# ShengkaiWu/IoU-aware-single-stage-object-detector

Measured on AMD Instinct MI355X. Metric: images/sec at 1333x800, IoU-aware RetinaNet R-50-FPN, higher is better.
Workload: dtype fp32; 1 GPU; IoU-aware RetinaNet R-50-FPN fp32, batch 8 per GPU, 3x800x1344 (1333x800 padded to /32), random-init weights, whole inference path incl. NMS, device-to-host copy and bbox2result (the reference's simple_test: per-class arrays on the host; batch i's host part runs under batch i+1's device part, the last one inside the timed region); global_batch=8, parallelism=dp1, dets_per_image=100

## Files before the change

### include/iouaware.h

```cpp
#ifndef IOUAWARE_H
#define IOUAWARE_H

#include <stddef.h>
#include <stdint.h>

#ifdef __cplusplus
extern "C" {
#endif

#define IA_MAX_LEVELS 8
#define IA_MAX_ANCHORS 16
#define IA_MAX_NMS_PRE 4096
#define IA_MAX_CANDIDATES 8192
#define IA_MAX_PER_IMG 1024

#define IA_F32 0
#define IA_BF16 1
#define IA_F16 2
#define IA_F64 3

#define IA_LAYOUT_NCHW 0
#define IA_LAYOUT_NHWC 1

#define IA_CLS_SIGMOID 0
// ... 53 lines not shown
                     int rescale, float *boxes, float *scores_t, float *best_score, void *stream);

size_t ia_multiclass_nms_workspace_bytes(int batch, int R, int C);
int ia_multiclass_nms(const float *boxes, const float *scores_t, const float *best_score,
                      int batch, int R, int C, float score_thr, float iou_thr, int max_per_img,
                      void *workspace, size_t workspace_bytes, float *dets, int32_t *labels,
                      int32_t *rows, int32_t *num, int32_t *keep_count, int32_t *keep_rows,
                      void *stream);

#define IA_SOFT_LINEAR 1
#define IA_SOFT_GAUSSIAN 2
size_t ia_multiclass_soft_nms_workspace_bytes(int batch, int R, int C);
int ia_multiclass_soft_nms(const float *boxes, const float *scores_t, int batch, int R, int C,
                           float score_thr, float iou_thr, int method, float sigma,
                           float min_score, int max_per_img, void *workspace,
                           size_t workspace_bytes, float *dets, int32_t *labels, int32_t *rows,
                           int32_t *num, int32_t *keep_count, int32_t *keep_rows, void *stream);

size_t ia_get_bboxes_workspace_bytes(const ia_head_geom *g, int batch);
size_t ia_get_bboxes_status_offset(const ia_head_geom *g, int batch);
int ia_debug_fused_spin_limit(int64_t limit);
int ia_profile_stage_events(void *begin, void *end);
int ia_get_bboxes(const ia_head_geom *g, const ia_level_ptrs *p, int batch, int dtype,
                  const float *img_hw, const float *scale_factor, int rescale, float score_thr,
                  float iou_thr, int max_per_img, void *workspace, size_t workspace_bytes,
                  float *dets, int32_t *labels, int32_t *rows, int32_t *num, void *stream);

int ia_get_bboxes_lazy(const ia_head_geom *g, const ia_level_ptrs *p, int batch, int dtype,
                       const float *img_hw, const float *scale_factor, int rescale,
                       float score_thr, float iou_thr, int max_per_img, int candidates,
                       void *workspace, size_t workspace_bytes, float *dets, int32_t *labels,
                       int32_t *rows, int32_t *num, void *stream);

size_t ia_multiclass_nms_lazy_workspace_bytes(int batch, int R, int C);
int ia_multiclass_nms_lazy(const float *boxes, const float *scores_t, const float *best_score,
                           int batch, int R, int C, float score_thr, float iou_thr,
                           int max_per_img, int candidates, void *workspace,
                           size_t workspace_bytes, float *dets, int32_t *labels, int32_t *rows,
                           int32_t *num, void *stream);

int ia_decode_stage(const ia_head_geom *g, const ia_level_ptrs *p, int batch, int dtype,
                    const float *img_hw, const float *scale_factor, int rescale, void *workspace,
                    size_t workspace_bytes, void *stream);

int ia_get_bboxes_workspace_layout(const ia_head_geom *g, int batch, size_t offsets[8]);

size_t ia_nms_workspace_bytes(int n);
int ia_nms(const float *dets, int n, float iou_thr, int32_t *keep, int32_t *count, void *workspace,
           size_t workspace_bytes, void *stream);

size_t ia_nms_f64_workspace_bytes(int n);
int ia_nms_f64(const double *dets, int n, float iou_thr, int32_t *keep, int32_t *count,
               void *workspace, size_t workspace_bytes, void *stream);

int ia_soft_nms(const float *dets, int n, float iou_thr, int method, float sigma, float min_score,
                float *out_dets, int32_t *out_inds, int32_t *count, void *stream);

typedef struct {
    const uint8_t *src;
    int32_t src_h, src_w, dst_h, dst_w, flip;
} ia_image_desc;
int ia_image_transform(const ia_image_desc *imgs, int batch, const float *mean, const float *std,
                       int to_rgb, int pad_h, int pad_w, int channels_last, float *out,
                       void *stream);

typedef struct {
    int32_t num_levels, batch;
    int32_t H[IA_MAX_LEVELS], W[IA_MAX_LEVELS];
} ia_wino_geom;
typedef struct {
    int32_t c0, n;
    int32_t dst_channels, dst_offset;
    float *dst[IA_MAX_LEVELS];
} ia_wino_seg;
int ia_wino_tiles(const ia_wino_geom *g, int32_t *tiles);
int ia_wino_input_transform(const ia_wino_geom *g, const float *const *x, int channels, int groups,
                            const float *pre_scale, const float *pre_shift, int pre_relu, float *V,
                            void *stream);
int ia_wino_output_transform(const ia_wino_geom *g, const float *M, int channels, int groups,
                             const float *bias, int relu, int nseg, const ia_wino_seg *segs,
                             void *stream);
int ia_wino_mid_transform(const ia_wino_geom *g, const float *M, int channels, int groups_m,
                          const float *bias, int relu, float *V, int groups_v, void *stream);

int ia_wino_grad_output_transform(const ia_wino_geom *g, const float *const *dy, int channels,
                                  float *dM, void *stream);

#define IA_COLSUM_MAX_STRIPS 512
size_t ia_relu_bwd_bias_grad_workspace_bytes(int64_t rows, int n);
int ia_wino_weight_transform(const float *w, int n_in, int n_out, int64_t stride_in,
                             int64_t stride_out, int64_t stride_ky, int64_t stride_kx, int flip,
                             const double *G, float *U, void *stream);
int ia_wino_weight_grad(const float *dU, int n_in, int n_out, const double *G, float *dW,
                        int64_t stride_in, int64_t stride_out, int64_t stride_ky, int64_t stride_kx,
                        void *stream);
int ia_bn_fold_fwd(const float *w, const float *gamma, const float *beta, const float *mean,
                   const float *inv_std, int cout, int K, float *w_out, float *b_out, void *stream);
int ia_bn_fold_bwd(const float *dw_folded, const float *db_folded, const float *w, const float *gamma,
                   const float *mean, const float *inv_std, int cout, int K, float *dw,
                   float *dgamma, float *dbeta, void *stream);
int ia_relu_bwd_bias_grad(const float *dy, const float *y, int64_t rows, int n, float *g, float *db,
                          void *workspace, size_t workspace_bytes, void *stream);

int ia_linear_bias_act(const float *A, const float *W, const float *bias, const float *residual,
                       float *D, int64_t rows, int k, int n, int relu, void *workspace,
                       size_t workspace_bytes, void *stream);
int ia_linear_bias_act_bf16(const void *A, const void *W, const float *bias, const void *residual,
                            void *D, int64_t rows, int k, int n, int relu, void *workspace,
                            size_t workspace_bytes, void *stream);
int ia_batched_gemm(const float *A, const float *W, float *D, int batch, int64_t rows, int k, int n,
                    void *workspace, size_t workspace_bytes, void *stream);
int ia_batched_gemm_stream(const float *A, const float *W, float *D, int batch, int64_t rows, int k,
                           int n, void *stream);

size_t ia_im2col3x3_bytes(int B, int H, int W, int C, int stride, int dtype);
int ia_im2col3x3_nhwc(const void *x, void *col, int B, int H, int W, int C, int stride, int dtype,
                      void *stream);
int ia_conv1x1_strided(const void *x, const void *W_kn, const float *bias, const void *residual,
                       void *D, int B, int H, int W, int k, int n, int stride, int relu, int dtype,
                       void *workspace, size_t workspace_bytes, void *stream);
int ia_col2im3x3_nhwc(const void *dcol, void *dx, int B, int H, int W, int C, int stride, int dtype,
                      void *stream);

int ia_gemm_tuning(int mode);

int ia_gemm_table_add(int64_t m, int64_t n, int64_t k, int flags, int batch, int dtype,
                      int solution_index);
int ia_gemm_table_clear(void);
int ia_gemm_table_dump(int64_t *rows7, int capacity);
int ia_gemm_table_stats(int64_t *hits_misses_stale);
int ia_gemm_library_version(void);

int ia_linear_bias_act_wt(const float *A, const float *W_nk, const float *bias,
                          const float *residual, float *D, int64_t rows, int k, int n, int relu,
                          void *workspace, size_t workspace_bytes, void *stream);
int ia_gemm_tn(const float *G, const float *X, float *D, int batch, int64_t rows, int n, int k,
               void *workspace, size_t workspace_bytes, void *stream);


int ia_focal_loss_fwd(const void *cls, int dtype, const int64_t *labels,
                      const float *label_weights, int B, int A, int C, int HW, float gamma,
                      float alpha, double *loss_sum, void *stream);
int ia_focal_loss_bwd(const void *cls, int dtype, const int64_t *labels,
                      const float *label_weights, int B, int A, int C, int HW, float gamma,
                      float alpha, float gscale, const float *gscale_dev, float *grad_cls,
                      void *stream);

int ia_smooth_l1_fwd(const void *pred, int dtype, const float *target, const float *weight,
                     int B, int A, int HW, float beta, double *loss_sum, void *stream);
int ia_smooth_l1_bwd(const void *pred, int dtype, const float *target, const float *weight,
                     int B, int A, int HW, float beta, float gscale, const float *gscale_dev,
                     float *grad_pred, void *stream);

int ia_balanced_l1_fwd(const void *pred, int dtype, const float *target, const float *weight,
                       int B, int A, int HW, float beta, float alpha, float gamma, double *loss_sum,
                       void *stream);
int ia_balanced_l1_bwd(const void *pred, int dtype, const float *target, const float *weight,
                       int B, int A, int HW, float beta, float alpha, float gamma, float gscale,
                       const float *gscale_dev, float *grad_pred, void *stream);

int ia_focal_loss_balanced_fwd(const void *cls, int dtype, const int64_t *labels,
                               const float *label_weights, const float *anchor_iou, int B, int A,
                               int C, int HW, float gamma, float alpha, float eta,
                               double *loss_sums3, void *stream);
int ia_focal_loss_balanced_bwd(const void *cls, int dtype, const int64_t *labels,
                               const float *label_weights, const float *anchor_iou, int B, int A,
// ... 343 lines not shown
```

### iou-aware-single-stage-object-detector_amd/csrc/wino.hip

```cpp
#include <string.h>
#include "ia_internal.hpp"
#include "ia_wino.hpp"

namespace ia {

typedef float f32x4_t __attribute__((ext_vector_type(4)));
__device__ __forceinline__ float4 load_nt(const float *p)
{
    const f32x4_t q = __builtin_nontemporal_load(reinterpret_cast<const f32x4_t *>(p));
    return make_float4(q.x, q.y, q.z, q.w);
}
__device__ __forceinline__ void store_nt(float *p, const float4 &v)
{
    f32x4_t q; q.x = v.x; q.y = v.y; q.z = v.z; q.w = v.w;
    __builtin_nontemporal_store(q, reinterpret_cast<f32x4_t *>(p));
}
__device__ __forceinline__ float4 f4(float v) { return make_float4(v, v, v, v); }
__device__ __forceinline__ float4 operator+(const float4 &a, const float4 &b) { return make_float4(a.x + b.x, a.y + b.y, a.z + b.z, a.w + b.w); }
__device__ __forceinline__ float4 operator-(const float4 &a, const float4 &b) { return make_float4(a.x - b.x, a.y - b.y, a.z - b.z, a.w - b.w); }
__device__ __forceinline__ float4 operator*(float s, const float4 &a) { return make_float4(s * a.x, s * a.y, s * a.z, s * a.w); }

__device__ __forceinline__ void bt6(const float4 (&d)[6], float4 (&o)[6])
{
    o[0] = (4.0f * d[0] - 5.0f * d[2]) + d[4];
// ... 40 lines not shown
    }
    return m;
}
static int tiles_per_wave(int channels)
{
    const int q = channels / 4;
    return (q < 64) ? (64 / q) : 1;
}

template <bool PACKED>
__global__ void __launch_bounds__(64) k_wino_in(WinoInArgs a)
{
    const LaneMap lm = lane_map<PACKED>(a.Ctot, a.T, a.tpw);
    if (!lm.on) return;
    const int t = lm.t, c = lm.c;
    int H, W;
    const TileRef r = locate_tile(a.lv, t, &H, &W);
    const float *x = level_ptr<!PACKED>(a.x, r.l) + (size_t)r.b * H * W * a.Ctot + c;
    const bool pre = a.pre_shift != nullptr;
    float4 ps = f4(1.0f), pb = f4(0.0f);
    if (pre) {
        if (a.pre_scale) ps = *reinterpret_cast<const float4 *>(a.pre_scale + c);
        pb = *reinterpret_cast<const float4 *>(a.pre_shift + c);
    }
    float4 d[6][6];
#pragma unroll
    for (int i = 0; i < 6; ++i) {
        const int y = r.y0 - 1 + i;
        const int yc = (y >= 0 && y < H) ? y : 0;
#pragma unroll
        for (int j = 0; j < 6; ++j) {
            const int xx = r.x0 - 1 + j;
            const int xc = (xx >= 0 && xx < W) ? xx : 0;
            d[i][j] = *reinterpret_cast<const float4 *>(x + ((size_t)yc * W + xc) * a.Ctot);
        }
    }
    if (pre) {
        const bool relu = a.pre_relu != 0;
#pragma unroll
        for (int i = 0; i < 6; ++i)
#pragma unroll
            for (int j = 0; j < 6; ++j) {
                float4 v = d[i][j];
                v = make_float4(v.x * ps.x + pb.x, v.y * ps.y + pb.y, v.z * ps.z + pb.z, v.w * ps.w + pb.w);
                const float4 z = make_float4(v.x > 0.f ? v.x : 0.f, v.y > 0.f ? v.y : 0.f,
                                             v.z > 0.f ? v.z : 0.f, v.w > 0.f ? v.w : 0.f);
                d[i][j] = relu ? z : v;
            }
    }
#pragma unroll
    for (int i = 0; i < 6; ++i) {
        const int y = r.y0 - 1 + i;
        const bool yin = (y >= 0) && (y < H);
#pragma unroll
        for (int j = 0; j < 6; ++j) {
            const int xx = r.x0 - 1 + j;
            const bool in = yin && (xx >= 0) && (xx < W);
            d[i][j] = in ? d[i][j] : f4(0.0f);
        }
    }
    float4 tmp[6][6];
#pragma unroll
    for (int j = 0; j < 6; ++j) {
        float4 col[6], o[6];
#pragma unroll
        for (int i = 0; i < 6; ++i) col[i] = d[i][j];
        bt6(col, o);
#pragma unroll
        for (int i = 0; i < 6; ++i) tmp[i][j] = o[i];
    }
    const int g = c / a.Cg, cc = c - g * a.Cg;
    float *v = a.V + ((size_t)g * 36 * a.T + t) * a.Cg + cc;
    const size_t kstride = (size_t)a.T * a.Cg;
#pragma unroll
    for (int i = 0; i < 6; ++i) {
        float4 o[6];
        bt6(tmp[i], o);
#pragma unroll
        for (int j = 0; j < 6; ++j)
            *reinterpret_cast<float4 *>(v + (size_t)(i * 6 + j) * kstride) = o[j];
    }
}

__device__ __forceinline__ void a6(const float4 (&y)[4], float4 (&o)[6])
{
    const float4 s02 = y[0] + y[2], s13 = y[1] + y[3];
    const float4 t02 = y[0] + 4.0f * y[2], t13 = 2.0f * y[1] + 8.0f * y[3];
    o[0] = y[0];
    o[1] = s02 + s13;
    o[2] = s02 - s13;
    o[3] = t02 + t13;
    o[4] = t02 - t13;
    o[5] = y[3];
}

template <bool PACKED>
__global__ void __launch_bounds__(64) k_wino_dy(WinoInArgs a)
{
    const LaneMap lm = lane_map<PACKED>(a.Ctot, a.T, a.tpw);
    if (!lm.on) return;
    const int t = lm.t, c = lm.c;
    int H, W;
    const TileRef r = locate_tile(a.lv, t, &H, &W);
    const float *x = level_ptr<!PACKED>(a.x, r.l) + (size_t)r.b * H * W * a.Ctot + c;
    float4 d[4][4];
#pragma unroll
    for (int i = 0; i < 4; ++i) {
        const int y = r.y0 + i;
        const int yc = (y < H) ? y : (H - 1);
#pragma unroll
        for (int j = 0; j < 4; ++j) {
            const int xx = r.x0 + j;
            const int xc = (xx < W) ? xx : (W - 1);
            const float4 v = *reinterpret_cast<const float4 *>(x + ((size_t)yc * W + xc) * a.Ctot);
            d[i][j] = (y < H && xx < W) ? v : f4(0.0f);
        }
    }
    float4 tmp[6][4];
#pragma unroll
    for (int j = 0; j < 4; ++j) {
        float4 col[4], o[6];
#pragma unroll
        for (int i = 0; i < 4; ++i) col[i] = d[i][j];
        a6(col, o);
#pragma unroll
        for (int i = 0; i < 6; ++i) tmp[i][j] = o[i];
    }
    const int g = c / a.Cg, cc = c - g * a.Cg;
    float *v = a.V + ((size_t)g * 36 * a.T + t) * a.Cg + cc;
    const size_t kstride = (size_t)a.T * a.Cg;
#pragma unroll
    for (int i = 0; i < 6; ++i) {
        float4 o[6];
        a6(tmp[i], o);
#pragma unroll
        for (int j = 0; j < 6; ++j)
            *reinterpret_cast<float4 *>(v + (size_t)(i * 6 + j) * kstride) = o[j];
    }
}

struct WinoOutArgs {
    WinoLevels lv;
    const float *M;
    const float *bias;
    WinoSeg seg[kMaxSeg];
    int32_t nseg, Ctot, Cg, T, relu, tpw;
};

template <bool PACKED>
__global__ void __launch_bounds__(64) k_wino_out(WinoOutArgs a)
{
    const LaneMap lm = lane_map<PACKED>(a.Ctot, a.T, a.tpw);
    if (!lm.on) return;
    const int t = lm.t, c = lm.c;
    int H, W;
    const TileRef r = locate_tile(a.lv, t, &H, &W);
    const int g = c / a.Cg, cc = c - g * a.Cg;
    const float *m = a.M + ((size_t)g * 36 * a.T + t) * a.Cg + cc;
    const size_t kstride = (size_t)a.T * a.Cg;
    float4 bz = f4(0.0f);
    if (a.bias) bz = *reinterpret_cast<const float4 *>(a.bias + c);
    float4 s[4][6];
#pragma unroll
    for (int j = 0; j < 6; ++j) {
        float4 col[6], o[4];
#pragma unroll
// ... 132 lines not shown
                    const int xx = 4 * txi + j, lx = lx0 + j;
                    float4 v = o[j] + bz;
                    if (a.relu) v = make_float4(v.x > 0.f ? v.x : 0.f, v.y > 0.f ? v.y : 0.f,
                                                v.z > 0.f ? v.z : 0.f, v.w > 0.f ? v.w : 0.f);
                    v = (y < H && xx < W) ? v : f4(0.0f);
                    if (ly >= 0 && ly < kMidP && lx >= 0 && lx < kMidP)
                        *reinterpret_cast<float4 *>(sy + (ly * kMidP + lx) * kMidCh) = v;
                }
            }
        } else {
#pragma unroll
            for (int i = 0; i < 4; ++i)
#pragma unroll
                for (int j = 0; j < 4; ++j) {
                    const int ly = ly0 + i, lx = lx0 + j;
                    if (ly >= 0 && ly < kMidP && lx >= 0 && lx < kMidP)
                        *reinterpret_cast<float4 *>(sy + (ly * kMidP + lx) * kMidCh) = f4(0.0f);
                }
        }
    }
    __syncthreads();

    const int tl = tid / kMidQ, tyl = tl / kMidB, txl = tl - tyl * kMidB;
    const int tyi = kMidB * byi + tyl, txi = kMidB * bxi + txl;
    if (tyi >= ty_n || txi >= tx) return;
    const float *sp = s_y + ((4 * tyl) * kMidP + 4 * txl) * kMidCh + cq;
    float4 tmp[6][6];
#pragma unroll
    for (int j = 0; j < 6; ++j) {
        float4 col[6], o[6];
#pragma unroll
        for (int i = 0; i < 6; ++i) col[i] = *reinterpret_cast<const float4 *>(sp + (i * kMidP + j) * kMidCh);
        bt6(col, o);
#pragma unroll
        for (int i = 0; i < 6; ++i) tmp[i][j] = o[i];
        __builtin_amdgcn_sched_barrier(0);
    }
    float *v = a.V + (size_t)gv * 36 * vstride + (size_t)(tbase + tyi * tx + txi) * a.Cv + (c - gv * a.Cv);
#pragma unroll
    for (int i = 0; i < 6; ++i) {
        float4 o[6];
        bt6(tmp[i], o);
#pragma unroll
        for (int j = 0; j < 6; ++j)
            *reinterpret_cast<float4 *>(v + (size_t)(i * 6 + j) * vstride) = o[j];
    }
}

}

extern "C" {

int ia_wino_tiles(const ia_wino_geom *g, int32_t *tiles)
{
    ia::WinoLevels w;
    int rc = ia::make_wino_levels(g, w);
    if (rc) return rc;
    if (tiles) *tiles = w.tile_off[w.L];
    return 0;
}

int ia_wino_input_transform(const ia_wino_geom *g, const float *const *x, int channels, int groups,
                            const float *pre_scale, const float *pre_shift, int pre_relu, float *V,
                            void *stream)
{
    ia::WinoInArgs a;
    int rc = ia::make_wino_levels(g, a.lv);
    if (rc) return rc;
    if (!x || !V || channels < 4 || (channels & 3) || groups < 1 || channels % groups) return IA_E_ARG;
    a.Ctot = channels; a.Cg = channels / groups; a.T = a.lv.tile_off[a.lv.L];
    if (a.Cg & 3) return IA_E_ARG;
    for (int l = 0; l < IA_MAX_LEVELS; ++l) {
        a.x[l] = (l < a.lv.L) ? x[l] : nullptr;
        if (l < a.lv.L && (!x[l] || ((uintptr_t)x[l] & 15u))) return IA_E_ARG;
    }
    a.V = V;
    if (pre_scale && !pre_shift) return IA_E_ARG;
    a.pre_scale = pre_scale; a.pre_shift = pre_shift; a.pre_relu = pre_relu ? 1 : 0;
    a.tpw = ia::tiles_per_wave(channels);
    const int waves = (a.T + a.tpw - 1) / a.tpw;
    dim3 grid((unsigned)((waves + 7) / 8 * 8), (unsigned)((channels / 4 + 63) / 64));
    if (a.tpw > 1) hipLaunchKernelGGL(ia::k_wino_in<true>, grid, dim3(64), 0, (hipStream_t)stream, a);
    else hipLaunchKernelGGL(ia::k_wino_in<false>, grid, dim3(64), 0, (hipStream_t)stream, a);
    return ia::hip_status(hipGetLastError());
}

int ia_wino_grad_output_transform(const ia_wino_geom *g, const float *const *dy, int channels,
                                   float *dM, void *stream)
{
    ia::WinoInArgs a;
    int rc = ia::make_wino_levels(g, a.lv);
    if (rc) return rc;
    if (!dy || !dM || channels < 4 || (channels & 3)) return IA_E_ARG;
    a.Ctot = channels; a.Cg = channels; a.T = a.lv.tile_off[a.lv.L];
    for (int l = 0; l < IA_MAX_LEVELS; ++l) {
        a.x[l] = (l < a.lv.L) ? dy[l] : nullptr;
        if (l < a.lv.L && (!dy[l] || ((uintptr_t)dy[l] & 15u))) return IA_E_ARG;
    }
    a.V = dM;
    a.pre_scale = a.pre_shift = nullptr; a.pre_relu = 0;
    a.tpw = ia::tiles_per_wave(channels);
    const int waves = (a.T + a.tpw - 1) / a.tpw;
    dim3 grid((unsigned)((waves + 7) / 8 * 8), (unsigned)((channels / 4 + 63) / 64));
    if (a.tpw > 1) hipLaunchKernelGGL(ia::k_wino_dy<true>, grid, dim3(64), 0, (hipStream_t)stream, a);
    else hipLaunchKernelGGL(ia::k_wino_dy<false>, grid, dim3(64), 0, (hipStream_t)stream, a);
    return ia::hip_status(hipGetLastError());
}

int ia_wino_output_transform(const ia_wino_geom *g, const float *M, int channels, int groups,
                             const float *bias, int relu, int nseg, const ia_wino_seg *segs,
                             void *stream)
{
    ia::WinoOutArgs a;
    int rc = ia::make_wino_levels(g, a.lv);
    if (rc) return rc;
    if (!M || channels < 4 || (channels & 3) || groups < 1 || channels % groups || !segs ||
        nseg < 1 || nseg > ia::kMaxSeg)
        return IA_E_ARG;
    a.M = M; a.bias = bias; a.Ctot = channels; a.Cg = channels / groups;
    if (a.Cg & 3) return IA_E_ARG;
    a.T = a.lv.tile_off[a.lv.L]; a.relu = relu ? 1 : 0; a.nseg = nseg;
    memset(a.seg, 0, sizeof(a.seg));
    for (int k = 0; k < nseg; ++k) {
        const ia_wino_seg &s = segs[k];
        if (s.c0 < 0 || s.n < 1 || s.c0 + s.n > channels || s.dst_channels < s.n + s.dst_offset ||
            s.dst_offset < 0)
            return IA_E_ARG;
        if (k > 0 && s.c0 < segs[k - 1].c0 + segs[k - 1].n) return IA_E_ARG;
        a.seg[k].c0 = s.c0; a.seg[k].n = s.n; a.seg[k].Cdst = s.dst_channels; a.seg[k].coff = s.dst_offset;
        for (int l = 0; l < a.lv.L; ++l) {
            if (!s.dst[l]) return IA_E_ARG;
            a.seg[k].dst[l] = s.dst[l];
        }
    }
    a.tpw = ia::tiles_per_wave(channels);
    const int waves = (a.T + a.tpw - 1) / a.tpw;
    dim3 grid((unsigned)((waves + 7) / 8 * 8), (unsigned)((channels / 4 + 63) / 64));
    if (a.tpw > 1) hipLaunchKernelGGL(ia::k_wino_out<true>, grid, dim3(64), 0, (hipStream_t)stream, a);
    else hipLaunchKernelGGL(ia::k_wino_out<false>, grid, dim3(64), 0, (hipStream_t)stream, a);
    return ia::hip_status(hipGetLastError());
}

int ia_wino_mid_transform(const ia_wino_geom *g, const float *M, int channels, int groups_m,
                          const float *bias, int relu, float *V, int groups_v, void *stream)
{
    ia::WinoMidArgs a;
    int rc = ia::make_wino_levels(g, a.lv);
    if (rc) return rc;
    if (!M || !V || channels < ia::kMidCh || groups_m < 1 || channels % groups_m || groups_v < 1 ||
        channels % groups_v)
        return IA_E_ARG;
    a.M = M; a.bias = bias; a.V = V; a.Ctot = channels;
    a.Cm = channels / groups_m; a.Cv = channels / groups_v;
    if (a.Cm % ia::kMidCh || a.Cv % ia::kMidCh || ((uintptr_t)M & 15u) || ((uintptr_t)V & 15u) ||
        ((uintptr_t)bias & 15u))
        return IA_E_ARG;
    a.T = a.lv.tile_off[a.lv.L]; a.relu = relu ? 1 : 0;
    int64_t n = 0;
    for (int l = 0; l < IA_MAX_LEVELS; ++l) {
        const bool on = l < a.lv.L;
        const int ty = on ? a.lv.tpi[l] / a.lv.tx[l] : 0;
        a.bx[l] = on ? (a.lv.tx[l] + ia::kMidB - 1) / ia::kMidB : 0;
        a.bpi[l] = on ? ((ty + ia::kMidB - 1) / ia::kMidB) * a.bx[l] : 0;
        a.blk_off[l] = (int32_t)n;
        n += (int64_t)a.lv.B * a.bpi[l];
    }
// ... 9 lines not shown
```

### iou-aware-single-stage-object-detector_amd/iouaware/_lib.py

```python
import ctypes as C
import os

IA_MAX_LEVELS = 8
IA_MAX_ANCHORS = 16
IA_MAX_NMS_PRE = 4096
IA_MAX_CANDIDATES = 8192
IA_MAX_PER_IMG = 1024
IA_F32, IA_BF16, IA_F16, IA_F64 = 0, 1, 2, 3
IA_LAYOUT_NCHW, IA_LAYOUT_NHWC = 0, 1
IA_CLS_SIGMOID, IA_CLS_SOFTMAX = 0, 1
IA_CLS_SIGMOID_NOIOU, IA_CLS_SOFTMAX_NOIOU = 2, 3
IA_LOSS_SLOTS = 64
IA_MAX_TARGET_BATCH = 16
IA_GN_CHUNK = 256

_CSRC = os.path.join(os.path.dirname(os.path.abspath(__file__)), '..', 'csrc')
SO_PATH = os.path.abspath(os.path.join(_CSRC, 'libiouaware_hip.so'))


class HeadGeom(C.Structure):
    _fields_ = [('num_levels', C.c_int32), ('num_anchors', C.c_int32),
                ('num_classes', C.c_int32), ('nms_pre', C.c_int32),
                ('H', C.c_int32 * IA_MAX_LEVELS), ('W', C.c_int32 * IA_MAX_LEVELS),
                ('stride', C.c_int32 * IA_MAX_LEVELS),
# ... 60 lines not shown
class PointLossCfg(C.Structure):
    _fields_ = [('gamma', C.c_float), ('alpha', C.c_float), ('attach_iou_target', C.c_int32),
                ('exact_large_logits', C.c_int32)]


class ImageDesc(C.Structure):
    _fields_ = [('src', C.c_void_p), ('src_h', C.c_int32), ('src_w', C.c_int32),
                ('dst_h', C.c_int32), ('dst_w', C.c_int32), ('flip', C.c_int32)]


class WinoGeom(C.Structure):
    _fields_ = [('num_levels', C.c_int32), ('batch', C.c_int32),
                ('H', C.c_int32 * IA_MAX_LEVELS), ('W', C.c_int32 * IA_MAX_LEVELS)]


class Conv3x3Desc(C.Structure):
    _fields_ = [('num_levels', C.c_int32), ('batch', C.c_int32), ('groups', C.c_int32),
                ('cin', C.c_int32), ('cout', C.c_int32), ('x_stride', C.c_int32), ('y_stride', C.c_int32),
                ('H', C.c_int32 * IA_MAX_LEVELS), ('W', C.c_int32 * IA_MAX_LEVELS),
                ('x', (C.c_void_p * IA_MAX_LEVELS) * 2), ('y', (C.c_void_p * IA_MAX_LEVELS) * 2)]


class WinoSeg(C.Structure):
    _fields_ = [('c0', C.c_int32), ('n', C.c_int32), ('dst_channels', C.c_int32),
                ('dst_offset', C.c_int32), ('dst', C.c_void_p * IA_MAX_LEVELS)]


_vp, _i, _f, _sz, _i64 = C.c_void_p, C.c_int, C.c_float, C.c_size_t, C.c_int64
_G, _P = C.POINTER(HeadGeom), C.POINTER(LevelPtrs)
_PG, _WG = C.POINTER(PointHeadGeom), C.POINTER(WinoGeom)
_PP, _PT, _PC = C.POINTER(PointLevelPtrs), C.POINTER(PointTargets), C.POINTER(PointLossCfg)
_PS = C.POINTER(PointPixStrides)

SIGNATURES = {
    'ia_version': (C.c_char_p, []),
    'ia_geom_sizes': (_i, [_G, C.POINTER(C.c_int32), C.POINTER(C.c_int32), C.POINTER(C.c_int32)]),
    'ia_decode_fuse_rowmax': (_i, [_G, _P, _i, _i, _vp, _vp]),
    'ia_select_topk_workspace_bytes': (_sz, [_G, _i]),
    'ia_select_topk': (_i, [_G, _vp, _i, _vp, _vp, _sz, _vp]),
    'ia_decode_fuse_rowmax_grouped': (_i, [_G, _P, _i, _i, _vp, _vp, _sz, _vp]),
    'ia_select_topk_grouped': (_i, [_G, _vp, _i, _vp, _vp, _sz, _vp]),
    'ia_decode_stage': (_i, [_G, _P, _i, _i, _vp, _vp, _i, _vp, _sz, _vp]),
    'ia_get_bboxes_status_offset': (_sz, [_G, _i]),
    'ia_debug_fused_spin_limit': (_i, [_i64]),
    'ia_profile_stage_events': (_i, [_vp, _vp]),
    'ia_gather_decode': (_i, [_G, _P, _i, _i, _vp, _vp, _vp, _i, _vp, _vp, _vp, _vp]),
    'ia_multiclass_nms_workspace_bytes': (_sz, [_i, _i, _i]),
    'ia_multiclass_nms': (_i, [_vp, _vp, _vp, _i, _i, _i, _f, _f, _i, _vp, _sz, _vp, _vp, _vp,
                               _vp, _vp, _vp, _vp]),
    'ia_multiclass_soft_nms_workspace_bytes': (_sz, [_i, _i, _i]),
    'ia_multiclass_soft_nms': (_i, [_vp, _vp, _i, _i, _i, _f, _f, _i, _f, _f, _i, _vp, _sz, _vp, _vp,
                                    _vp, _vp, _vp, _vp, _vp]),
    'ia_soft_nms': (_i, [_vp, _i, _f, _i, _f, _f, _vp, _vp, _vp, _vp]),
    'ia_get_bboxes_workspace_bytes': (_sz, [_G, _i]),
    'ia_get_bboxes': (_i, [_G, _P, _i, _i, _vp, _vp, _i, _f, _f, _i, _vp, _sz, _vp, _vp, _vp,
                           _vp, _vp]),
    'ia_multiclass_nms_lazy_workspace_bytes': (_sz, [_i, _i, _i]),
    'ia_multiclass_nms_lazy': (_i, [_vp, _vp, _vp, _i, _i, _i, _f, _f, _i, _i, _vp, _sz, _vp, _vp, _vp,
                                    _vp, _vp]),
    'ia_get_bboxes_lazy': (_i, [_G, _P, _i, _i, _vp, _vp, _i, _f, _f, _i, _i, _vp, _sz, _vp, _vp, _vp,
                                _vp, _vp]),
    'ia_get_bboxes_workspace_layout': (_i, [_G, _i, C.POINTER(_sz * 8)]),
    'ia_nms_workspace_bytes': (_sz, [_i]),
    'ia_nms': (_i, [_vp, _i, _f, _vp, _vp, _vp, _sz, _vp]),
    'ia_nms_f64_workspace_bytes': (_sz, [_i]),
    'ia_nms_f64': (_i, [_vp, _i, _f, _vp, _vp, _vp, _sz, _vp]),
    'ia_image_transform': (_i, [C.POINTER(ImageDesc), _i, C.POINTER(C.c_float), C.POINTER(C.c_float),
                                _i, _i, _i, _i, _vp, _vp]),
    'ia_wino_tiles': (_i, [C.POINTER(WinoGeom), C.POINTER(C.c_int32)]),
    'ia_wino_input_transform': (_i, [C.POINTER(WinoGeom), C.POINTER(C.c_void_p), _i, _i, _vp, _vp, _i,
                                     _vp, _vp]),
    'ia_wino_grad_output_transform': (_i, [C.POINTER(WinoGeom), C.POINTER(C.c_void_p), _i, _vp, _vp]),
    'ia_wino_weight_transform': (_i, [_vp, _i, _i, C.c_int64, C.c_int64, C.c_int64, C.c_int64, _i,
                                      C.POINTER(C.c_double), _vp, _vp]),
    'ia_wino_weight_grad': (_i, [_vp, _i, _i, C.POINTER(C.c_double), _vp, C.c_int64, C.c_int64,
                                 C.c_int64, C.c_int64, _vp]),
    'ia_bn_fold_fwd': (_i, [_vp, _vp, _vp, _vp, _vp, _i, _i, _vp, _vp, _vp]),
    'ia_bn_fold_bwd': (_i, [_vp, _vp, _vp, _vp, _vp, _vp, _i, _i, _vp, _vp, _vp, _vp]),
    'ia_relu_bwd_bias_grad_workspace_bytes': (C.c_size_t, [C.c_int64, _i]),
    'ia_relu_bwd_bias_grad': (_i, [_vp, _vp, C.c_int64, _i, _vp, _vp, _vp, C.c_size_t, _vp]),
    'ia_wino_output_transform': (_i, [C.POINTER(WinoGeom), _vp, _i, _i, _vp, _i, _i,
                                      C.POINTER(WinoSeg), _vp]),
    'ia_wino_mid_transform': (_i, [C.POINTER(WinoGeom), _vp, _i, _i, _vp, _i, _vp, _i, _vp]),
    'ia_linear_bias_act': (_i, [_vp, _vp, _vp, _vp, _vp, _i64, _i, _i, _i, _vp, _sz, _vp]),
    'ia_linear_bias_act_bf16': (_i, [_vp, _vp, _vp, _vp, _vp, _i64, _i, _i, _i, _vp, _sz, _vp]),
    'ia_batched_gemm': (_i, [_vp, _vp, _vp, _i, _i64, _i, _i, _vp, _sz, _vp]),
    'ia_batched_gemm_stream': (_i, [_vp, _vp, _vp, _i, _i64, _i, _i, _vp]),
    'ia_linear_bias_act_wt': (_i, [_vp, _vp, _vp, _vp, _vp, _i64, _i, _i, _i, _vp, _sz, _vp]),
    'ia_gemm_tuning': (_i, [_i]),
    'ia_im2col3x3_bytes': (_sz, [_i, _i, _i, _i, _i, _i]),
    'ia_im2col3x3_nhwc': (_i, [_vp, _vp, _i, _i, _i, _i, _i, _i, _vp]),
    'ia_col2im3x3_nhwc': (_i, [_vp, _vp, _i, _i, _i, _i, _i, _i, _vp]),
    'ia_conv1x1_strided': (_i, [_vp, _vp, _vp, _vp, _vp, _i, _i, _i, _i, _i, _i, _i, _i, _vp, _sz, _vp]),
    'ia_gemm_table_add': (_i, [_i64, _i64, _i64, _i, _i, _i, _i]),
    'ia_gemm_table_clear': (_i, []),
    'ia_gemm_table_dump': (_i, [_vp, _i]),
    'ia_gemm_table_stats': (_i, [_vp]),
    'ia_gemm_library_version': (_i, []),
    'ia_gemm_tn': (_i, [_vp, _vp, _vp, _i, _i64, _i, _i, _vp, _sz, _vp]),
    'ia_focal_loss_fwd': (_i, [_vp, _i, _vp, _vp, _i, _i, _i, _i, _f, _f, _vp, _vp]),
    'ia_focal_loss_bwd': (_i, [_vp, _i, _vp, _vp, _i, _i, _i, _i, _f, _f, _f, _vp, _vp, _vp]),
    'ia_smooth_l1_fwd': (_i, [_vp, _i, _vp, _vp, _i, _i, _i, _f, _vp, _vp]),
    'ia_smooth_l1_bwd': (_i, [_vp, _i, _vp, _vp, _i, _i, _i, _f, _f, _vp, _vp, _vp]),
    'ia_balanced_l1_fwd': (_i, [_vp, _i, _vp, _vp, _i, _i, _i, _f, _f, _f, _vp, _vp]),
    'ia_balanced_l1_bwd': (_i, [_vp, _i, _vp, _vp, _i, _i, _i, _f, _f, _f, _f, _vp, _vp, _vp]),
    'ia_focal_loss_balanced_fwd': (_i, [_vp, _i, _vp, _vp, _vp, _i, _i, _i, _i, _f, _f, _f, _vp, _vp]),
    'ia_focal_loss_balanced_bwd': (_i, [_vp, _i, _vp, _vp, _vp, _i, _i, _i, _i, _f, _f, _f, _vp, _f,
                                        _vp, _vp, _vp]),
    'ia_smooth_l1_balanced_fwd': (_i, [_vp, _i, _vp, _vp, _vp, _i, _i, _i, _f, _f, _vp, _vp]),
    'ia_smooth_l1_balanced_bwd': (_i, [_vp, _i, _vp, _vp, _vp, _i, _i, _i, _f, _f, _f, _vp, _vp,
                                       _vp]),
    'ia_iou_bce_fwd': (_i, [_G, _i, _vp, _vp, _i, _vp, _vp, _i, _vp, _vp, _vp]),
    'ia_iou_bce_bwd': (_i, [_G, _i, _vp, _vp, _i, _vp, _vp, _i, _f, _vp, _vp, _vp, _vp]),
    'ia_anchor_targets': (_i, [_G, _vp, _vp, _vp, _i, _i, _vp, _f, _f, _f, _f, _vp, _vp, _vp, _vp,
                               _vp, _vp, _vp]),
    'ia_anchor_targets_ptrs': (_i, [_G, C.POINTER(C.c_void_p), C.POINTER(C.c_void_p),
                                    C.POINTER(C.c_int32), _i, C.POINTER(C.c_int32), _f, _f, _f, _f,
                                    _vp, _vp, _vp, _vp, _vp, _vp, _vp]),
    'ia_head_loss_workspace_bytes': (_sz, [_G, _i]),
    'ia_head_loss_workspace_bytes_cfg': (_sz, [_G, _i, C.POINTER(HeadLossCfg)]),
    'ia_head_loss_fwd': (_i, [_G, _P, _i, _i, C.POINTER(HeadTargets), C.POINTER(HeadLossCfg), _vp,
                              _sz, _vp, _vp]),
    'ia_head_loss_bwd': (_i, [_G, _P, _i, _i, C.POINTER(HeadTargets), C.POINTER(HeadLossCfg), _vp,
                              _vp, _vp, _P, _vp]),
    'ia_head_loss_fwd_nhwc': (_i, [_G, _P, C.POINTER(LevelPixStrides), _i, C.POINTER(HeadTargets),
                                   C.POINTER(HeadLossCfg), _vp, _sz, _vp, _vp]),
    'ia_head_loss_bwd_nhwc': (_i, [_G, _P, C.POINTER(LevelPixStrides), _i, C.POINTER(HeadTargets),
                                   C.POINTER(HeadLossCfg), _vp, _vp, _P, C.POINTER(LevelPixStrides),
                                   _vp]),
    'ia_head_loss_fwd_box': (_i, [_G, _P, _i, _i, C.POINTER(HeadTargets), C.POINTER(HeadLossCfg),
                                  C.POINTER(BoxLossCfg), _vp, _sz, _vp, _vp]),
    'ia_head_loss_bwd_box': (_i, [_G, _P, _i, _i, C.POINTER(HeadTargets), C.POINTER(HeadLossCfg),
                                  C.POINTER(BoxLossCfg), _vp, _vp, _vp, _P, _vp]),
    'ia_head_loss_fwd_nhwc_box': (_i, [_G, _P, C.POINTER(LevelPixStrides), _i, C.POINTER(HeadTargets),
                                       C.POINTER(HeadLossCfg), C.POINTER(BoxLossCfg), _vp, _sz, _vp, _vp]),
    'ia_head_loss_bwd_nhwc_box': (_i, [_G, _P, C.POINTER(LevelPixStrides), _i, C.POINTER(HeadTargets),
                                       C.POINTER(HeadLossCfg), C.POINTER(BoxLossCfg), _vp, _vp, _P,
                                       C.POINTER(LevelPixStrides), _vp]),
    'ia_grouped_conv3x3_pack': (_i, [_vp, _vp, _i, _i, _vp]),
    'ia_grouped_conv3x3_nhwc': (_i, [_vp, _vp, _vp, _vp, _i, _i, _i, _i, _i, _i, _i, _vp]),
    'ia_grouped_conv3x3_packed_bytes_bf16': (C.c_size_t, [_i, _i]),
    'ia_grouped_conv3x3_pack_dev': (_i, [_vp, _vp, _i, _i, _i, _vp, _vp]),
    'ia_grouped_conv3x3_bwd_data_nhwc': (_i, [_vp, _vp, _vp, _i, _i, _i, _i, _i, _i, _vp]),
    'ia_grouped_conv3x3_bwd_weight_workspace_bytes': (C.c_size_t, [_i, _i, _i, _i, _i, _i]),
    'ia_grouped_conv3x3_bwd_weight_nhwc': (_i, [_vp, _vp, _vp, _vp, C.c_size_t, _i, _i, _i, _i, _i, _i, _vp]),
    'ia_grouped_conv3x3_pack_bf16': (_i, [_vp, _vp, _i, _i, _vp]),
    'ia_grouped_conv3x3_bf16_nhwc': (_i, [_vp, _vp, _vp, _vp, _i, _i, _i, _i, _i, _i, _i, _vp]),
    'ia_sigmoid_focal_loss_fwd': (_i, [_vp, _vp, _i, _i, _f, _f, _vp, _vp]),
    'ia_sigmoid_focal_loss_bwd': (_i, [_vp, _vp, _vp, _i, _i, _f, _f, _vp, _vp]),
    'ia_sigmoid_focal_loss_fwd_dt': (_i, [_vp, _i, _vp, _i, _i, _f, _f, _vp, _vp]),
    'ia_sigmoid_focal_loss_bwd_dt': (_i, [_vp, _i, _vp, _vp, _i, _i, _f, _f, _vp, _vp]),
    'ia_channel_affine_act': (_i, [_vp, _i, _vp, _vp, _vp, _vp, _vp, _i, _i, _i, _i64, _vp]),
    'ia_channel_affine_act_nhwc': (_i, [_vp, _i, _vp, _vp, _vp, _vp, _vp, _i, _i64, _i, _vp]),
    'ia_nhwc_to_nchw': (_i, [_vp, _vp, _i, _i, _i, _i64, _vp]),
    'ia_upsample2x_add_nhwc': (_i, [_vp, _vp, _i, _i, _i, _i, _i, _i, _vp]),
    'ia_conv1x1_stream': (_i, [_vp, _vp, _vp, _vp, _vp, C.c_int64, _i, _i, _i, _vp]),
    'ia_stem_conv7x7s2': (_i, [_vp, _vp, _vp, _i, _i, _i, _vp]),
    'ia_stem_conv7x7s2_bf16': (_i, [_vp, _vp, _vp, _i, _i, _i, _vp]),
    'ia_conv1x1_wide': (_i, [_vp, _vp, _vp, _vp, _vp, C.c_int64, _i, _i, _i, _vp]),
    'ia_conv1x1_chain': (_i, [_vp, _vp, _vp, _vp, _vp, _vp, _vp, _vp, _i64, _i, _i, _i, _vp]),
    'ia_conv3x3_bf16_packed_bytes': (C.c_size_t, [_i, _i, _i]),
    'ia_conv3x3_bf16_pack': (_i, [_vp, _i, _i, _i, _vp, _vp]),
    'ia_conv3x3_bf16_levels': (_i, [_vp, _vp, _vp, _i, _vp]),
    'ia_conv3x3_bf16_wgrad_workspace_bytes': (C.c_size_t, [_vp]),
    'ia_conv3x3_bf16_wgrad_plan': (_i, [_vp, C.POINTER(C.c_int32), C.POINTER(C.c_int32), C.POINTER(C.c_int32)]),
    'ia_conv3x3_bf16_wgrad_levels': (_i, [_vp, _vp, _vp, C.c_size_t, _vp]),
# ... 96 lines not shown
```

### iou-aware-single-stage-object-detector_amd/iouaware/winograd.py

```python
import collections
import ctypes as C

import numpy as np
import torch

from . import _lib
from .ops import _ptr, _stream, stream_id

_G = np.array([[1 / 4, 0, 0], [-1 / 6, -1 / 6, -1 / 6], [-1 / 6, 1 / 6, -1 / 6],
               [1 / 24, 1 / 12, 1 / 6], [1 / 24, -1 / 12, 1 / 6], [0, 0, 1]], dtype=np.float64)


_G_DEV = {}


def transform_weight(w):
    if w.dim() != 4 or w.shape[2] != 3 or w.shape[3] != 3:
        raise ValueError('Winograd F(4,3) needs a 3x3 kernel, got %s' % (tuple(w.shape),))
    g = w.detach().to(torch.float64)
    G = _G_DEV.get(g.device)
    if G is None:
        G = _G_DEV[g.device] = torch.from_numpy(_G).to(g.device)
    u = torch.einsum('ik,ockl,jl->ijco', G, g, G)
    return u.reshape(36, g.shape[1], g.shape[0]).to(torch.float32).contiguous()
# ... 61 lines not shown
    def acts(self, name, channels):
        key = ('acts', name, channels)
        a = self._bufs.get(key)
        if a is None:
            a = [torch.empty((self.batch, channels, h, w), dtype=torch.float32, device=self.device,
                             memory_format=torch.channels_last) for (h, w) in self.sizes]
            self._bufs[key] = a
        return a


TIMING = None


def _timed(kind, nbytes, launch):
    if TIMING is None:
        return launch()
    e0, e1 = torch.cuda.Event(enable_timing=True), torch.cuda.Event(enable_timing=True)
    e0.record()
    launch()
    e1.record()
    TIMING.append((kind, e0, e1, nbytes))


def input_transform(plan, xs, groups, out, pre=None):
    ptrs = (C.c_void_p * len(xs))(*[x.data_ptr() for x in xs])
    ps, pb, pr = pre if pre is not None else (None, None, False)
    ch = int(xs[0].shape[1])
    _timed('in', plan.T * ch * 4 * (16 + 36), lambda: _lib.check(
        _lib.lib().ia_wino_input_transform(C.byref(plan.geom), ptrs, ch, int(groups), _ptr(ps),
                                           _ptr(pb), int(bool(pr)), _ptr(out), _stream()),
        'ia_wino_input_transform'))
    return out


def output_transform(plan, m, channels, groups, bias, relu, segments):
    segs = (_lib.WinoSeg * len(segments))()
    for k, (c0, n, dst, off) in enumerate(segments):
        segs[k].c0, segs[k].n = int(c0), int(n)
        segs[k].dst_channels, segs[k].dst_offset = int(dst[0].shape[1]), int(off)
        for l, t in enumerate(dst):
            segs[k].dst[l] = t.data_ptr()
    _timed('out', plan.T * int(channels) * 4 * (36 + 16), lambda: _lib.check(
        _lib.lib().ia_wino_output_transform(C.byref(plan.geom), _ptr(m), int(channels), int(groups),
                                            _ptr(bias), int(bool(relu)), len(segments), segs,
                                            _stream()), 'ia_wino_output_transform'))


MID_CHANNELS = 32


def mid_transform(plan, m, channels, groups_m, bias, relu, out, groups_v):
    _timed('mid', plan.T * int(channels) * 4 * (36 + 36), lambda: _lib.check(
        _lib.lib().ia_wino_mid_transform(C.byref(plan.geom), _ptr(m), int(channels), int(groups_m),
                                         _ptr(bias), int(bool(relu)), _ptr(out), int(groups_v),
                                         _stream()), 'ia_wino_mid_transform'))
    return out


_LT_WS_BYTES = 128 << 20


STREAM_BMM = True
_STREAM_BMM_SHAPES = ((64, 64),)


def batched_gemm(v, u, out):
    from . import ops
    ops._ensure_gemm_table()
    batch, rows, k = v.shape
    n = u.shape[2]
    if not (v.is_contiguous() and u.is_contiguous() and out.is_contiguous()):
        raise ValueError('batched_gemm needs contiguous stacks')
    if STREAM_BMM and (k, n) in _STREAM_BMM_SHAPES and rows >= 4096 and v.dtype == torch.float32:
        _lib.check(_lib.lib().ia_batched_gemm_stream(_ptr(v), _ptr(u), _ptr(out), int(batch), int(rows),
                                                     int(k), int(n), _stream()), 'ia_batched_gemm_stream')
        return out
    ws = _scratch(v.device, 'lt_ws', (_LT_WS_BYTES // 4,))
    _lib.check(_lib.lib().ia_batched_gemm(_ptr(v), _ptr(u), _ptr(out), int(batch), int(rows), int(k),
                                          int(n), _ptr(ws), _LT_WS_BYTES, _stream()),
               'ia_batched_gemm')
    return out


class WinogradConv3x3(object):

    def __init__(self, weight, bias, relu=False):
        self.u = transform_weight(weight)
        self.bias = None if bias is None else bias.detach().to(torch.float32).contiguous()
        self.relu = relu
        self.cin, self.cout = self.u.shape[1], self.u.shape[2]
        if self.cout % 4:
            raise ValueError('output channels must be a multiple of 4')
        self._plans = collections.OrderedDict()

    def usable(self, x):
        return _usable(x) and x.shape[1] == self.cin \
            and not (torch.is_grad_enabled() and x.requires_grad)

    def __call__(self, x, pre=None):
        key = (x.shape[0], tuple(x.shape[-2:]), x.device, stream_id())
        plan = _plan_for(self._plans, key, lambda: _Plan([tuple(x.shape[-2:])], x.shape[0], x.device))
        v = input_transform(plan, [x], 1, plan.buf('v', (36, plan.T, self.cin)), pre)
        m = batched_gemm(v, self.u, plan.buf('m', (36, plan.T, self.cout)))
        y = torch.empty((x.shape[0], self.cout) + tuple(x.shape[-2:]), dtype=torch.float32,
                        device=x.device, memory_format=torch.channels_last)
        output_transform(plan, m, self.cout, 1, self.bias, self.relu, [(0, self.cout, [y], 0)])
        return y


def plain_3x3(conv):
    return (tuple(conv.kernel_size) == (3, 3) and tuple(conv.stride) == (1, 1)
            and tuple(conv.padding) == (1, 1) and tuple(conv.dilation) == (1, 1) and conv.groups == 1)


def _pair(a, b, F, granule):
    na, nb = a.out_channels, (0 if b is None else b.out_channels)
    n_pad = (na + nb + granule - 1) // granule * granule
    dev = a.weight.device
    u = torch.zeros((36, F, n_pad), dtype=torch.float32, device=dev)
    u[:, :, :na] = transform_weight(a.weight)
    bias = torch.zeros(n_pad, dtype=torch.float32, device=dev)
    bias[:na] = a.bias.detach().float()
    if b is not None:
        u[:, :, na:na + nb] = transform_weight(b.weight)
        bias[na:na + nb] = b.bias.detach().float()
    return u.contiguous(), bias.contiguous(), na, nb


class _WinogradTowers(object):

    FUSE_MID = True
    mid_bias = None

    def __init__(self, head):
        convs_c, convs_r = list(head.cls_convs), list(head.reg_convs)
        self.n_layers = len(convs_c)
        F = head.feat_channels
        if head.in_channels % 4 or F % 4:
            raise ValueError('channel counts must be multiples of 4')
        self.F, self.cin = F, head.in_channels
        self.u0 = torch.cat([transform_weight(convs_c[0].conv.weight),
                             transform_weight(convs_r[0].conv.weight)], dim=2).contiguous()
        self.u = [torch.cat([transform_weight(convs_c[i].conv.weight),
                             transform_weight(convs_r[i].conv.weight)], dim=0).contiguous()
                  for i in range(1, self.n_layers)]
        self._plans = collections.OrderedDict()

    def usable(self, feats):
        return all(_usable(x) and x.shape[1] == self.cin for x in feats) \
            and not torch.is_grad_enabled()

    def _towers(self, feats):
        B, dev = feats[0].shape[0], feats[0].device
        sizes = [tuple(x.shape[-2:]) for x in feats]
        key = (B, tuple(sizes), dev, stream_id())
        plan = _plan_for(self._plans, key, lambda: _Plan(sizes, B, dev))
        T, F = plan.T, self.F
        v = input_transform(plan, feats, 1, plan.buf('v', (36, T, self.cin)))
        m = batched_gemm(v, self.u0, plan.buf('m', (36, T, 2 * F)))
        new = lambda c: [torch.empty((B, c, h, w), dtype=torch.float32, device=dev,
                                     memory_format=torch.channels_last) for (h, w) in sizes]
        if self.FUSE_MID and self.mid_bias is not None and F % MID_CHANNELS == 0:
            groups = 1
            for i, u in enumerate(self.u):
                v = mid_transform(plan, m, 2 * F, groups, self.mid_bias[i], True,
                                  plan.buf('v', (72, T, F)), 2)
                m = batched_gemm(v, u, plan.buf('m', (72, T, F)))
                groups = 2
            v = mid_transform(plan, m, 2 * F, groups, self.mid_bias[self.n_layers - 1], True,
                              plan.buf('v', (72, T, F)), 2)
            return plan, v, new
        acts = plan.acts('a', 2 * F)
        self._layer_out(plan, m, 1, 0, acts)
        for i, u in enumerate(self.u):
            v = input_transform(plan, acts, 2, plan.buf('v', (72, T, F)))
            m = batched_gemm(v, u, plan.buf('m', (72, T, F)))
            nxt = plan.acts('b' if acts is plan.acts('a', 2 * F) else 'a', 2 * F)
            self._layer_out(plan, m, 2, i + 1, nxt)
            acts = nxt
        v = input_transform(plan, acts, 2, plan.buf('v', (72, T, F)))
        return plan, v, new

    @staticmethod
    def _out_conv(plan, v, name, u, bias, segments):
        n = u.shape[2]
        m = batched_gemm(v, u, plan.buf(name, (36, plan.T, n)))
# ... 92 lines not shown
```

Baseline: 407.7 img/s.

## Fuse Winograd input transform with batched GEMM for 64-channel 3x3 convs

Adds a HIP kernel that computes the Winograd F(4,3) input transform for 16 tiles into double-buffered LDS and multiplies it straight away against fragment-packed transformed weights with fp32 MFMA, writing M directly. The intermediate V tensor (36 x T x 64) is no longer written to and read back from global memory, and one kernel launch goes away. The trade-offs are more LDS use and register pressure per block, and a hand-written GEMM that may be slower than the tuned streaming bmm. The path applies only to 64-in/64-out convs with at least 4096 tiles, which in R-50 are the layer1 3x3 convs.

```diff
diff --git a/include/iouaware.h b/include/iouaware.h
--- a/include/iouaware.h
+++ b/include/iouaware.h
@@ -159,6 +159,8 @@
                              void *stream);
 int ia_wino_mid_transform(const ia_wino_geom *g, const float *M, int channels, int groups_m,
                           const float *bias, int relu, float *V, int groups_v, void *stream);
+int ia_wino_in_gemm(const ia_wino_geom *g, const float *const *x, int channels, const float *pre_scale,
+                    const float *pre_shift, int pre_relu, const float *u_packed, float *M, void *stream);
 
 int ia_wino_grad_output_transform(const ia_wino_geom *g, const float *const *dy, int channels,
                                   float *dM, void *stream);
diff --git a/iou-aware-single-stage-object-detector_amd/csrc/wino.hip b/iou-aware-single-stage-object-detector_amd/csrc/wino.hip
--- a/iou-aware-single-stage-object-detector_amd/csrc/wino.hip
+++ b/iou-aware-single-stage-object-detector_amd/csrc/wino.hip
@@ -146,6 +146,159 @@
     }
 }
 
+struct WinoInGemmArgs {
+    WinoLevels lv;
+    const float *x[IA_MAX_LEVELS];
+    const float *U;
+    float *M;
+    const float *pre_scale, *pre_shift;
+    int32_t T, pre_relu, ngroups;
+};
+
+template <int C>
+__global__ void __launch_bounds__(4 * C) k_wino_in_gemm(WinoInGemmArgs a)
+{
+    static_assert(C == 64, "lane maps and the LDS swizzle are worked out for 16 quads per tile");
+    constexpr int Q = C / 4, TPW = 64 / Q, NB = C / 16, J = C / 16;
+    constexpr int kPlane = 16 * C;
+    __shared__ __attribute__((aligned(16))) float s_v[2 * 6 * kPlane];
+    const int grp = xcd_tile(blockIdx.x, a.ngroups);
+    if (grp >= a.ngroups) return;
+    const int lane = threadIdx.x & 63;
+    const int wave = __builtin_amdgcn_readfirstlane(threadIdx.x >> 6);
+
+    const int sub = lane / Q, quad = lane - sub * Q, tg = wave * TPW + sub, c = 4 * quad;
+    const int t0 = grp * 16 + tg;
+    const int t = t0 < a.T ? t0 : a.T - 1;
+    int H, W;
+    const TileRef r = locate_tile(a.lv, t, &H, &W);
+    const float *x = level_ptr<false>(a.x, r.l) + (size_t)r.b * H * W * C + c;
+    const bool pre = a.pre_shift != nullptr;
+    float4 ps = f4(1.0f), pb = f4(0.0f);
+    if (pre) {
+        if (a.pre_scale) ps = *reinterpret_cast<const float4 *>(a.pre_scale + c);
+        pb = *reinterpret_cast<const float4 *>(a.pre_shift + c);
+    }
+    float4 d[6][6];
+#pragma unroll
+    for (int i = 0; i < 6; ++i) {
+        const int y = r.y0 - 1 + i;
+        const int yc = (y >= 0 && y < H) ? y : 0;
+#pragma unroll
+        for (int j = 0; j < 6; ++j) {
+            const int xx = r.x0 - 1 + j;
+            const int xc = (xx >= 0 && xx < W) ? xx : 0;
+            d[i][j] = *reinterpret_cast<const float4 *>(x + ((size_t)yc * W + xc) * C);
+        }
+    }
+    if (pre) {
+        const bool relu = a.pre_relu != 0;
+#pragma unroll
+        for (int i = 0; i < 6; ++i)
+#pragma unroll
+            for (int j = 0; j < 6; ++j) {
+                float4 v = d[i][j];
+                v = make_float4(v.x * ps.x + pb.x, v.y * ps.y + pb.y, v.z * ps.z + pb.z, v.w * ps.w + pb.w);
+                const float4 z = make_float4(v.x > 0.f ? v.x : 0.f, v.y > 0.f ? v.y : 0.f,
+                                             v.z > 0.f ? v.z : 0.f, v.w > 0.f ? v.w : 0.f);
+                d[i][j] = relu ? z : v;
+            }
+    }
+#pragma unroll
+    for (int i = 0; i < 6; ++i) {
+        const int y = r.y0 - 1 + i;
+        const bool yin = (y >= 0) && (y < H);
+#pragma unroll
+        for (int j = 0; j < 6; ++j) {
+            const int xx = r.x0 - 1 + j;
+            const bool in = yin && (xx >= 0) && (xx < W);
+            d[i][j] = in ? d[i][j] : f4(0.0f);
+        }
+    }
+    float4 tmp[6][6];
+#pragma unroll
+    for (int j = 0; j < 6; ++j) {
+        float4 col[6], o[6];
+#pragma unroll
+        for (int i = 0; i < 6; ++i) col[i] = d[i][j];
+        bt6(col, o);
+#pragma unroll
+        for (int i = 0; i < 6; ++i) tmp[i][j] = o[i];
+    }
+    float *const sw = s_v + tg * C + 4 * (quad ^ tg);
+
+    const int p = lane & 15, q = lane >> 4;
+    const int tp = grp * 16 + p;
+    const bool live = tp < a.T;
+    const float *const sr = s_v + p * C;
+    int xo[J];
+#pragma unroll
+    for (int j = 0; j < J; ++j) xo[j] = 4 * ((4 * j + q) ^ p);
+    const float *const up = a.U + ((size_t)wave * J * 64 + lane) * 4;
+    float *const mp = a.M + ((size_t)(live ? tp : 0) * C + 16 * wave + 4 * q);
+    const size_t kstride = (size_t)a.T * C;
+
+    constexpr int PG = 2;
+    f32x4_t wn[PG][J];
+#pragma unroll
+    for (int g = 0; g < PG; ++g)
+#pragma unroll
+        for (int j = 0; j < J; ++j) wn[g][j] = *reinterpret_cast<const f32x4_t *>(up + g * (C * C) + j * 256);
+
+    {
+        float4 o[6];
+        bt6(tmp[0], o);
+#pragma unroll
+        for (int j = 0; j < 6; ++j) *reinterpret_cast<float4 *>(sw + j * kPlane) = o[j];
+    }
+    __syncthreads();
+#pragma unroll
+    for (int i = 0; i < 6; ++i) {
+        if (i + 1 < 6) {
+            float4 o[6];
+            bt6(tmp[i + 1], o);
+            float *const s = sw + ((i + 1) & 1) * 6 * kPlane;
+#pragma unroll
+            for (int j = 0; j < 6; ++j) *reinterpret_cast<float4 *>(s + j * kPlane) = o[j];
+        }
+#pragma unroll
+        for (int j6 = 0; j6 < 6; j6 += PG) {
+            const int k = i * 6 + j6;
+            const float *const s = sr + ((i & 1) * 6 + j6) * kPlane;
+            f32x4_t xv[PG][J], wv[PG][J], acc[PG];
+#pragma unroll
+            for (int g = 0; g < PG; ++g) {
+#pragma unroll
+                for (int j = 0; j < J; ++j) {
+                    xv[g][j] = *reinterpret_cast<const f32x4_t *>(s + g * kPlane + xo[j]);
+                    wv[g][j] = wn[g][j];
+                }
+                acc[g] = f32x4_t{0.0f, 0.0f, 0.0f, 0.0f};
+            }
+            if (k + PG < 36) {
+                const float *const un = up + (size_t)(k + PG) * (C * C);
+#pragma unroll
+                for (int g = 0; g < PG; ++g)
+#pragma unroll
+                    for (int j = 0; j < J; ++j) wn[g][j] = *reinterpret_cast<const f32x4_t *>(un + g * (C * C) + j * 256);
+            }
+            __builtin_amdgcn_sched_barrier(0);
+#pragma unroll
+            for (int j = 0; j < J; ++j)
+#pragma unroll
+                for (int cc = 0; cc < 4; ++cc)
+#pragma unroll
+                    for (int g = 0; g < PG; ++g)
+                        acc[g] = __builtin_amdgcn_mfma_f32_16x16x4f32(wv[g][j][cc], xv[g][j][cc], acc[g], 0, 0, 0);
+            if (live) {
+#pragma unroll
+                for (int g = 0; g < PG; ++g) *reinterpret_cast<f32x4_t *>(mp + (size_t)(k + g) * kstride) = acc[g];
+            }
+        }
+        if (i + 1 < 6) __syncthreads();
+    }
+}
+
 __device__ __forceinline__ void a6(const float4 (&y)[4], float4 (&o)[6])
 {
     const float4 s02 = y[0] + y[2], s13 = y[1] + y[3];
@@ -444,6 +597,30 @@
     dim3 grid((unsigned)((waves + 7) / 8 * 8), (unsigned)((channels / 4 + 63) / 64));
     if (a.tpw > 1) hipLaunchKernelGGL(ia::k_wino_in<true>, grid, dim3(64), 0, (hipStream_t)stream, a);
     else hipLaunchKernelGGL(ia::k_wino_in<false>, grid, dim3(64), 0, (hipStream_t)stream, a);
+    return ia::hip_status(hipGetLastError());
+}
+
+int ia_wino_in_gemm(const ia_wino_geom *g, const float *const *x, int channels, const float *pre_scale,
+                    const float *pre_shift, int pre_relu, const float *u_packed, float *M, void *stream)
+{
+    ia::WinoInGemmArgs a;
+    int rc = ia::make_wino_levels(g, a.lv);
+    if (rc) return rc;
+    if (!x || !u_packed || !M || channels != 64) return IA_E_ARG;
+    if (((uintptr_t)u_packed & 15u) || ((uintptr_t)M & 15u) || ((uintptr_t)pre_scale & 15u) ||
+        ((uintptr_t)pre_shift & 15u))
+        return IA_E_ARG;
+    for (int l = 0; l < IA_MAX_LEVELS; ++l) {
+        a.x[l] = (l < a.lv.L) ? x[l] : nullptr;
+        if (l < a.lv.L && (!x[l] || ((uintptr_t)x[l] & 15u))) return IA_E_ARG;
+    }
+    if (pre_scale && !pre_shift) return IA_E_ARG;
+    a.U = u_packed; a.M = M;
+    a.pre_scale = pre_scale; a.pre_shift = pre_shift; a.pre_relu = pre_relu ? 1 : 0;
+    a.T = a.lv.tile_off[a.lv.L];
+    a.ngroups = (int32_t)(((int64_t)a.T + 15) / 16);
+    dim3 grid((unsigned)((a.ngroups + 7) / 8 * 8));
+    hipLaunchKernelGGL(ia::k_wino_in_gemm<64>, grid, dim3(256), 0, (hipStream_t)stream, a);
     return ia::hip_status(hipGetLastError());
 }
 
diff --git a/iou-aware-single-stage-object-detector_amd/iouaware/_lib.py b/iou-aware-single-stage-object-detector_amd/iouaware/_lib.py
--- a/iou-aware-single-stage-object-detector_amd/iouaware/_lib.py
+++ b/iou-aware-single-stage-object-detector_amd/iouaware/_lib.py
@@ -166,6 +166,7 @@
     'ia_wino_output_transform': (_i, [C.POINTER(WinoGeom), _vp, _i, _i, _vp, _i, _i,
                                       C.POINTER(WinoSeg), _vp]),
     'ia_wino_mid_transform': (_i, [C.POINTER(WinoGeom), _vp, _i, _i, _vp, _i, _vp, _i, _vp]),
+    'ia_wino_in_gemm': (_i, [C.POINTER(WinoGeom), C.POINTER(C.c_void_p), _i, _vp, _vp, _i, _vp, _vp, _vp]),
     'ia_linear_bias_act': (_i, [_vp, _vp, _vp, _vp, _vp, _i64, _i, _i, _i, _vp, _sz, _vp]),
     'ia_linear_bias_act_bf16': (_i, [_vp, _vp, _vp, _vp, _vp, _i64, _i, _i, _i, _vp, _sz, _vp]),
     'ia_batched_gemm': (_i, [_vp, _vp, _vp, _i, _i64, _i, _i, _vp, _sz, _vp]),
diff --git a/iou-aware-single-stage-object-detector_amd/iouaware/winograd.py b/iou-aware-single-stage-object-detector_amd/iouaware/winograd.py
--- a/iou-aware-single-stage-object-detector_amd/iouaware/winograd.py
+++ b/iou-aware-single-stage-object-detector_amd/iouaware/winograd.py
@@ -167,10 +167,34 @@
     return out
 
 
+FUSE_IN_GEMM = True
+_IN_GEMM_CHANNELS = (64,)
+
+
+def pack_u_fragments(u):
+    b, k, n = u.shape
+    if k % 16 or n % 16:
+        raise ValueError('fragment order needs multiples of 16 channels')
+    return u.reshape(b, k // 16, 4, 4, n // 16, 16).permute(0, 4, 1, 2, 5, 3).contiguous() \
+            .view(b, n // 16, k // 16, 64, 4)
+
+
+def input_transform_gemm(plan, xs, u_packed, out, pre=None):
+    ptrs = (C.c_void_p * len(xs))(*[x.data_ptr() for x in xs])
+    ps, pb, pr = pre if pre is not None else (None, None, False)
+    _lib.check(_lib.lib().ia_wino_in_gemm(C.byref(plan.geom), ptrs, int(xs[0].shape[1]), _ptr(ps), _ptr(pb),
+                                          int(bool(pr)), _ptr(u_packed), _ptr(out), _stream()),
+               'ia_wino_in_gemm')
+    return out
+
+
 class WinogradConv3x3(object):
 
     def __init__(self, weight, bias, relu=False):
         self.u = transform_weight(weight)
+        self.u_packed = None
+        if self.u.shape[1] == self.u.shape[2] and self.u.shape[1] in _IN_GEMM_CHANNELS:
+            self.u_packed = pack_u_fragments(self.u)
         self.bias = None if bias is None else bias.detach().to(torch.float32).contiguous()
         self.relu = relu
         self.cin, self.cout = self.u.shape[1], self.u.shape[2]
@@ -185,8 +209,13 @@
     def __call__(self, x, pre=None):
         key = (x.shape[0], tuple(x.shape[-2:]), x.device, stream_id())
         plan = _plan_for(self._plans, key, lambda: _Plan([tuple(x.shape[-2:])], x.shape[0], x.device))
-        v = input_transform(plan, [x], 1, plan.buf('v', (36, plan.T, self.cin)), pre)
-        m = batched_gemm(v, self.u, plan.buf('m', (36, plan.T, self.cout)))
+        if (FUSE_IN_GEMM and self.u_packed is not None and STREAM_BMM
+                and (self.cin, self.cout) in _STREAM_BMM_SHAPES and plan.T >= 4096
+                and x.dtype == torch.float32):
+            m = input_transform_gemm(plan, [x], self.u_packed, plan.buf('m', (36, plan.T, self.cout)), pre)
+        else:
+            v = input_transform(plan, [x], 1, plan.buf('v', (36, plan.T, self.cin)), pre)
+            m = batched_gemm(v, self.u, plan.buf('m', (36, plan.T, self.cout)))
         y = torch.empty((x.shape[0], self.cout) + tuple(x.shape[-2:]), dtype=torch.float32,
                         device=x.device, memory_format=torch.channels_last)
         output_transform(plan, m, self.cout, 1, self.bias, self.relu, [(0, self.cout, [y], 0)])
```

After: 412.8 img/s (median of 6 runs). 1.01x the previous value.
